# BAMresearch/McSAS

Hardware: AMD Instinct MI355X
Metric: MC accept/reject steps/sec (whole node) (higher is better)
Workload: dtype f64; 1 GPU; Sphere, synthetic 512 q-points x 400 contribs, 50 reps on this rank (50 in all), 20000 MC steps per chain per launch, convergenceCriterion=0, one analysis on the chip at a time; reps_total=50, reps_per_gpu=50, ranks_seen=1, streams=1, exec_mode=pipeline, waves_per_chain=1, q_per_lane=8, window=192, launches=108, cached_rows=True

## Files before the change

mcsas_amd/csrc/pipe_layout.h:

```cpp
#pragma once
#include "chain_common.h"

namespace mcsas {

struct PipeSnap {
    int32_t attempt, t_init, alive, pad;
    uint64_t init_base;
    uint64_t step_base;
};

struct PipeChain {
    PipeSnap snap[2];
    double SC, SIC, SCC, A, b, chi2;
    double X;
    int64_t num_iter, num_moves, total_steps;
    uint64_t draw_pos, t_start;
    int32_t attempts, converged, stopped, overflow, done, pad;
#ifdef MCSAS_STAMPS
    int64_t dbg[20];
    uint64_t last_end;
#endif
};

struct PipeGeom {
    int32_t kb;
    int32_t w;
    int32_t rows_per_wave;
    int32_t prod_blocks_y;
    int32_t scan_waves;
    int32_t qpl;
    int32_t gram_off;
    int32_t sub_per_block;
    int32_t lazy_rows;
    int32_t overlap;
    int32_t gram_lds;
    int32_t drow_off;
    int32_t resum_every;
    int32_t rowq;
    int32_t rec_off;
    int32_t help;
    uint64_t prod_lds, scan_lds;
};

struct PipeArgs {
    ChainArgs c;
    PipeGeom g;
    PipeChain *chains;
    double *ft, *wft;
    int32_t *slot_of;
    int32_t *stage_slot;
    double *dwin;
    double *gwin;
    double *scal;
    int32_t *row_valid;
    double *pval;
    int32_t *povf;
    int32_t *rowq;
    int32_t *n_done;
    int32_t *n_done_dev;
    int32_t tick, pad;
    uint64_t *timeline;
    int32_t timeline_tick, pad1;
};

struct PipeHot {
    const double *q, *w, *wI, *q3inv;
    PipeChain *chains;
    int32_t n_reps, n_contrib, n_active, qpad, kb, prod_blocks_y, w_sub, pad;
    int64_t max_iter;
};

constexpr int PIPE_BLOCK = 512;
constexpr int PIPE_WAVES = PIPE_BLOCK / 64;
constexpr int PIPE_GRAM_TILES_PER_ROUND = 2;
constexpr int PIPE_DROW_PAD = 8;
constexpr int PIPE_GRAM_NT_MAX = 3;
constexpr int PIPE_RESUM_STEPS = 64;
constexpr int PIPE_MAX_ROW_DOUBLES = 32;
#define PIPE_TL_WORDS 30

static inline int pipe_geometry(int nq, int n_contrib, int tab_doubles, int heavy_rows, int rows_per_wave_req, int sub_req, int gram_global_req, int eager_req, int n_chains, int n_cus, PipeGeom *g,
                                int contrib_doubles) {
    int qpl = 1;
    while (qpl * 64 < nq) qpl *= 2;
    if (qpl > 16) return 1;
    const int qpad = qpl * 64;
    g->rowq = 0; g->rec_off = 0; g->help = 0;
    if (heavy_rows) {
        int kb = (n_contrib / 2) & ~7;
        int cap = PIPE_BLOCK;
#ifndef __HIPCC_RTC__
        if (const char *e = getenv("MCSAS_HIP_PIPE_KB_CAP")) { const int v = atoi(e) & ~7; if (v >= 8 && v <= PIPE_BLOCK) cap = v; }
#endif
        if (kb > cap) kb = cap;
        if (n_chains > 0 && n_cus > 0) {
            const double slots = 8.0 * (double)n_cus;
            auto rate = [&](int c) { const double r = (double)n_chains * c / slots; return (double)c / (0.75 + (double)(long long)(r + 1.0 - 1e-9)); };
            const double rmax = (double)n_chains * kb / slots;
            if (rmax > 2.0 && rmax < 4.0) {
                int best = kb;
                double best_v = rate(kb);
                for (int c = kb - 8; c >= 8 && 2 * c >= kb; c -= 8)
                    if (rate(c) > best_v * 1.02) { best_v = rate(c); best = c; }
                kb = best;
            }
        }
#ifndef __HIPCC_RTC__
        if (const char *e = getenv("MCSAS_HIP_PIPE_KB")) { const int v = atoi(e) & ~7; if (v >= 8 && v <= ((n_contrib / 2) & ~7) && v <= cap) kb = v; }
#endif
        if (kb < 8) return 1;
        int by = 8;
        if (n_chains > 0 && n_cus > 0) { by = (n_cus + n_chains - 1) / n_chains; if (by < 1) by = 1; if (by > 32) by = 32; if (by * 8 > kb) by = (kb + 7) / 8; }
        g->kb = kb; g->qpl = qpl; g->w = 8; g->sub_per_block = 1; g->rows_per_wave = 1; g->prod_blocks_y = by;
        g->gram_off = 4 * qpad + tab_doubles; g->resum_every = PIPE_RESUM_STEPS;
        g->overlap = 0; g->gram_lds = 0; g->drow_off = 0; g->lazy_rows = 0;
        g->rowq = 1; g->rec_off = g->gram_off + 16;
        const size_t rec = (size_t)kb * (contrib_doubles + MCSAS_MAX_ACTIVE + 2) + ((size_t)3 * kb + 1) / 2;
        g->prod_lds = sizeof(double) * ((size_t)g->rec_off + rec);
        g->help = (n_chains > 1 && (size_t)n_chains <= 2 * rec) ? 1 : 0;
#ifndef __HIPCC_RTC__
        if (const char *e = getenv("MCSAS_HIP_PIPE_HELP")) g->help = atoi(e) ? g->help : 0;
#endif
        g->scan_waves = PIPE_WAVES;
        g->scan_lds = sizeof(double) * ((size_t)g->w * qpad + 2 * (size_t)g->w * g->w + 3 * (size_t)qpad + (size_t)g->kb * 4 + 64)
                    + sizeof(int32_t) * (4 * (size_t)g->kb + 1 + 1 + 64 + 4 + 8) + 64;
        if (g->scan_lds > 160 * 1024 || g->prod_lds > 160 * 1024) return 2;
        return 0;
    }
    const bool overlap = gram_global_req;
    auto pick_w = [&](int r) {
        int w = 8;
        for (int ws = 8; ws <= 8 * r && ws <= (overlap ? 32 : 64); ws += 8) {
            const int rps = ws / 8;
            if (rps == 5 || rps == 7 || rps * qpl > PIPE_MAX_ROW_DOUBLES) continue;
            if ((8 * r) % ws == 0 && sizeof(double) * (size_t)ws * qpad <= 96 * 1024 && (sub_req == 0 || ws <= 8 * sub_req)) w = ws;
        }
        return w;
    };
    int rpw = 0, by = 0;
    if (rows_per_wave_req >= 1 && rows_per_wave_req <= 8) {
        rpw = rows_per_wave_req;
        while (rpw > 1 && 2 * 8 * rpw > n_contrib) --rpw;
        if (2 * 8 * rpw > n_contrib) return 1;
        by = n_contrib / (2 * 8 * rpw);
        if (by * 8 * rpw > 256) by = 256 / (8 * rpw);
    } else {
        static const int order[6] = {6, 8, 4, 3, 2, 1};
        int kbs[6], best_kb = 0;
        for (int c = 0; c < 6; ++c) {
            const int r = order[c];
            int b = (2 * 8 * r > n_contrib) ? 0 : n_contrib / (2 * 8 * r);
            if (b * 8 * r > 256) b = 256 / (8 * r);
            kbs[c] = b * 8 * r;
            if (kbs[c] > best_kb) best_kb = kbs[c];
        }
        if (best_kb == 0) return 1;
        int rpw_d = 0, by_d = 0;
        for (int c = 0; c < 6 && !rpw_d; ++c)
            if (kbs[c] > 0 && 20 * kbs[c] >= 17 * best_kb) { rpw_d = order[c]; by_d = kbs[c] / (8 * rpw_d); }
        if (n_chains > 0 && n_cus > 0) {
            static const int small_first[6] = {3, 4, 6, 8, 2, 1};
            for (int c = 0; c < 6 && !rpw; ++c) {
                const int r = small_first[c];
                int b = (2 * 8 * r > n_contrib) ? 0 : n_contrib / (2 * 8 * r);
                if (b * 8 * r > 256) b = 256 / (8 * r);
                if (b > 0 && b * 8 * r == by_d * 8 * rpw_d && pick_w(r) == pick_w(rpw_d) && n_chains * (b + 1) <= n_cus) { rpw = r; by = b; }
            }
        }
        if (!rpw) { rpw = rpw_d; by = by_d; }
    }
    g->kb = by * 8 * rpw; g->qpl = qpl;
    g->w = pick_w(rpw);
    g->sub_per_block = 8 * rpw / g->w;
    g->rows_per_wave = rpw;
    g->prod_blocks_y = by;
    g->gram_off = 4 * qpad + tab_doubles;
    g->resum_every = 0;
    {
        const size_t red = overlap ? (size_t)2 * PIPE_WAVES * PIPE_GRAM_NT_MAX * 256 : (size_t)PIPE_WAVES * PIPE_GRAM_TILES_PER_ROUND * 256;
        g->prod_lds = sizeof(double) * ((size_t)g->gram_off + 16 + red);
        g->overlap = overlap ? 1 : 0;
        g->gram_lds = 0; g->drow_off = 0;
        const size_t with_rows = g->prod_lds + sizeof(double) * (size_t)g->w * (qpad + PIPE_DROW_PAD);
        if (!overlap && with_rows <= 160 * 1024) {
            g->gram_lds = 1; g->drow_off = g->gram_off + 16 + (int)red; g->prod_lds = with_rows;
        }
        g->lazy_rows = ((g->gram_lds || overlap) && !eager_req) ? 1 : 0;
        if (!g->gram_lds && !g->overlap) return 2;
#ifndef MCSAS_TUNING
        if (g->overlap) return 2;
#endif
    }
    g->scan_waves = PIPE_WAVES;
    g->scan_lds = sizeof(double) * ((size_t)g->w * qpad + 2 * (size_t)g->w * g->w + 2 * (size_t)qpad + (size_t)g->kb * 4 + 64)
                + sizeof(int32_t) * (4 * (size_t)g->kb + 1 + 1 + 64 + 4 + 8) + 64;
    if (g->scan_lds > 160 * 1024 || g->prod_lds > 160 * 1024) return 2;
    return 0;
}

}
```

mcsas_amd/csrc/pipe_prod.h:

```cpp
#pragma once
#include "pipe_rowq.h"
#include <type_traits>

namespace mcsas {

#define PIPE_PIN_ROW(arr) do { _Pragma("unroll") for (int j_ = 0; j_ < QPL; ++j_) asm volatile("" : "+v"(arr[j_])); } while (0)

#ifdef MCSAS_STAMPS
#define PIPE_TL_SLOT(pa, i) (pa).timeline[((size_t)blockIdx.x * 8 + (threadIdx.x >> 6)) * PIPE_TL_WORDS + 4 + (i)]
#define PIPE_TL_PUT(pa, t, i, val) do { if ((pa).timeline && (t) - 1 == (pa).timeline_tick && (threadIdx.x & 63) == 0) PIPE_TL_SLOT(pa, i) = (val); } while (0)
#define PIPE_TL_CLOCK(var) const uint64_t var = wall_clock64()
#else
#define PIPE_TL_PUT(pa, t, i, val) do {} while (0)
#define PIPE_TL_CLOCK(var) do {} while (0)
#endif
#define PIPE_TL_WRITE(pa, t, i) PIPE_TL_PUT(pa, t, i, wall_clock64())
#define PIPE_TLX_MARK(pa, t, i) PIPE_TL_WRITE(pa, t, 18 + (i))
#define PIPE_TL_MARK(pa, t, i) PIPE_TL_WRITE(pa, t, i)

template <int M> constexpr bool pipe_light_model_v = Contrib<M>::ROW_CLASS == 0;
template <int M>
__device__ __forceinline__ double pipe_point_intensity(const Contrib<M> &c, double q, double q3inv, const double *tab) {
    if constexpr (M == MCSAS_MODEL_SPHERE) return c.fast ? c.intensity_fast(q, q3inv) : c.intensity(q, tab);
    else return c.intensity(q, tab);
}

template <int QPL>
__device__ __forceinline__ void load_row_pairs(const MCSAS_GLOBAL double *row, int lane, double (&r)[QPL]) {
    if constexpr (QPL >= 2) {
#pragma unroll
        for (int c = 0; c < QPL / 2; ++c) {
            const v2f64 v = *(const MCSAS_GLOBAL v2f64 *)(row + 128 * c + 2 * lane);
            r[2 * c] = v.x; r[2 * c + 1] = v.y;
        }
    } else {
        r[0] = row[lane];
    }
}
template <int QPL>
__device__ __forceinline__ void load_row_pairs_lds(const double *row, int lane, double (&r)[QPL]) {
    if constexpr (QPL >= 2) {
#pragma unroll
        for (int c = 0; c < QPL / 2; ++c) {
            const v2f64 v = *reinterpret_cast<const v2f64 *>(row + 128 * c + 2 * lane);
            r[2 * c] = v.x; r[2 * c + 1] = v.y;
        }
    } else {
        r[0] = row[lane];
    }
}

template <int M, int QPL, bool RQ>
__device__ __forceinline__ void pipe_prod_block(const PipeArgs &pa, const PipeHot &hot, double *lds, int rep, int by, int gy, int t) {
    const ChainArgs &a = pa.c;
    const int tid = threadIdx.x, lane = tid & 63, wave = tid >> 6;
    constexpr int WPB = PIPE_BLOCK / 64;
    const int N = hot.n_contrib, P = hot.n_active, qpad = hot.qpad, Kb = hot.kb;
    const int64_t max_iter = hot.max_iter;
    constexpr int QTB = (QPL * 64 + PIPE_BLOCK - 1) / PIPE_BLOCK;
    double tq[QTB], tw[QTB], twI[QTB], tq3[QTB];
#pragma unroll
    for (int x = 0; x < QTB; ++x) {
        const int i = tid + PIPE_BLOCK * x < qpad ? tid + PIPE_BLOCK * x : 0;
        tq[x] = glb(hot.q)[i]; tw[x] = glb(hot.w)[i]; twI[x] = glb(hot.wI)[i]; tq3[x] = glb(hot.q3inv)[i];
    }
    PIPE_TL_CLOCK(c_entry);
    const PipeSnap sn = load_snap(&hot.chains[rep].snap[t & 1]);
    const bool own = sn.alive && t >= sn.t_init;
    if (!own && !(RQ && pa.g.help)) return;
    PIPE_TL_CLOCK(c_snap);

    double *lq = lds, *lw = lds + qpad, *lwI = lds + 2 * qpad, *lq3 = lds + 3 * qpad, *tab = lds + 4 * qpad;
#pragma unroll
    for (int x = 0; x < QTB; ++x) {
        const int i = tid + PIPE_BLOCK * x;
        if (i < qpad) { lq[i] = tq[x]; lw[i] = tw[x]; lwI[i] = twI[x]; lq3[i] = tq3[x]; }
    }
    PIPE_TL_CLOCK(c_tab);
    Contrib<M>::fill_table(a.model, tab, tid, PIPE_BLOCK);
    if (tid == 0) *reinterpret_cast<int32_t *>(lds + pa.g.gram_off + 16) = 0;
    __syncthreads();
    PIPE_TL_CLOCK(c_bar);
    PIPE_TL_PUT(pa, t, 22, c_entry); PIPE_TL_PUT(pa, t, 23, c_snap); PIPE_TL_PUT(pa, t, 24, c_tab); PIPE_TL_PUT(pa, t, 25, c_bar);
    const QTables qt = make_qtables<M>(a.model, lq, lq3, tab);
    if constexpr (RQ) { pipe_prod_rowq<M, QPL>(pa, hot, lds, qt, rep, by, gy, t, sn, own); return; }
    auto rset = glb(a.rset) + (size_t)rep * N * P;
    auto cache = glb(a.cache) + (size_t)rep * a.cache_rows * qpad;
    const DrawSource src{a.replay ? a.replay + (size_t)rep * a.replay_len : nullptr, a.replay_len, a.seed,
                         (uint32_t)(a.rep_offset + rep)};
    auto slot_of = glb(pa.slot_of) + (size_t)rep * N;
    auto stage = glb(pa.stage_slot) + (size_t)rep * 2 * Kb;
    auto row_valid = glb(pa.row_valid) + (size_t)rep * N;
    const int gw = by * WPB + wave, nw = gy * WPB;

    if (t == sn.t_init) {
        for (int i = tid + by * PIPE_BLOCK; i < N; i += PIPE_BLOCK * gy) { slot_of[i] = i; row_valid[i] = 1; }
        for (int i = tid + by * PIPE_BLOCK; i < 2 * Kb; i += PIPE_BLOCK * gy) stage[i] = N + i;
        int ovf = 0;
        for (int nb = 0; nb < N; nb += nw * WAVE) {
            const int n = nb + lane * nw + gw;
            double row[MCSAS_MAX_ACTIVE] = {0., 0., 0., 0.};
            if (n < N) {
#pragma unroll
                for (int p = 0; p < MCSAS_MAX_ACTIVE; ++p)
                    if (p < P) {
                        if (a.start_from_min) row[p] = a.start_value[p];
                        else {
                            double u = src.at(sn.init_base + (uint64_t)p * N + n, ovf);
                            row[p] = gen_transform(a.gen_kind[p], u) * (a.gen_hi[p] - a.gen_lo[p]) + a.gen_lo[p];
                        }
                        rset[(size_t)n * P + p] = row[p];
                    }
            } else {
#pragma unroll
                for (int p = 0; p < MCSAS_MAX_ACTIVE; ++p) row[p] = a.gen_lo[p] > 0. ? a.gen_lo[p] : 1e-9;
            }
            Contrib<M> mine;
            mine.prepare(a.model, row);
            for (int l = 0; l < WAVE; ++l) {
                const int nn = nb + l * nw + gw;
                if (nn >= N) break;
                const Contrib<M> c = mine.bcast(__builtin_amdgcn_readfirstlane(l));
                double it[QPL];
                RowEval<M, QPL>::run(c, qt, lane, it);
#pragma unroll
                for (int j = 0; j < QPL; ++j) cache[(size_t)nn * qpad + lane + WAVE * j] = it[j];
            }
        }
        if (__any(ovf) && lane == 0) atomicOr(&pa.chains[rep].overflow, 1);
        return;
    }

    if (MCSAS_TUNE_BITS(a) & 16) return;
    if constexpr (pipe_light_model_v<M>) if (pa.g.overlap || pa.g.gram_lds) {
        const int W = pa.g.w, nsb = pa.g.sub_per_block, BR = nsb * W;
        const int rw_even = W >> 3, skew_bits = (MCSAS_TUNE_BITS(a) >> 19) & 3;
        const int skew_req = pa.g.gram_lds ? (skew_bits == 0 ? 1 : (skew_bits == 3 ? 0 : skew_bits)) : skew_bits;
        const int skew = skew_req < rw_even ? skew_req : rw_even - 1;
        const int wv = __builtin_amdgcn_readfirstlane(wave);
        const int RW = wv < 4 ? rw_even + skew : rw_even - skew;
        const int rbase = wv < 4 ? wv * (rw_even + skew) : 4 * (rw_even + skew) + (wv - 4) * (rw_even - skew);
        const int buf = t & 1;
        const int64_t w = (int64_t)t - sn.t_init - 1;
        const int64_t sb0 = w * Kb + (int64_t)by * BR;
        auto dwin = glb(pa.dwin) + ((size_t)rep * 2 + buf) * Kb * qpad;
        auto scal = glb(pa.scal) + ((size_t)rep * 2 + buf) * Kb * 4;
        auto pval = glb(pa.pval) + ((size_t)rep * 2 + buf) * Kb * MCSAS_MAX_ACTIVE;
        auto povf = glb(pa.povf) + ((size_t)rep * 2 + buf) * Kb;
        auto gwin = glb(pa.gwin) + ((size_t)rep * 2 + buf) * Kb * W;
        double *gred = lds + pa.g.gram_off + 16;
        constexpr size_t GRED = (size_t)PIPE_WAVES * PIPE_GRAM_NT_MAX * 256;
        const int nmine = nsb * RW;
        const bool no_gram = MCSAS_TUNE_BITS(a) & 64;
        const int lrow = (lane / RW) * W + rbase + (lane % RW);
        const bool lazy = pa.g.lazy_rows;
        PIPE_TLX_MARK(pa, t, 0);
        constexpr int CON = 12;
        static_assert(sizeof(Contrib<M>) <= 8 * CON && sizeof(Contrib<M>) % 8 == 0, "Contrib record");
        int32_t *stl = reinterpret_cast<int32_t *>(gred);
        double *scon = gred + 64;
        double prow[MCSAS_MAX_ACTIVE] = {0., 0., 0., 0.};
        const int l2 = lane - 32;
        const bool old_lane = lazy && l2 >= 0 && l2 < nmine;
        int stale_r = -1;
        if (old_lane) {
            const int lrow_o = (l2 / RW) * W + rbase + (l2 % RW);
            if (sb0 + lrow_o < max_iter) {
                const int r = (int)((sb0 + lrow_o) % N);
                const int v = row_valid[r];
#pragma unroll
                for (int p = 0; p < MCSAS_MAX_ACTIVE; ++p) if (p < P) prow[p] = rset[(size_t)r * P + p];
                if (!v) stale_r = r;
            }
        }
        int pov = 0, my_oslot = 0, my_sslot = 0;
        {
            const int r = (int)((sb0 + lrow) % N);
            if (lane < nmine) {
                if (lazy) my_oslot = r;
                else { my_oslot = slot_of[r]; my_sslot = stage[buf * Kb + by * BR + lrow]; }
            }
            const int64_t sl = sb0 + lrow;
#pragma unroll
            for (int p = 0; p < MCSAS_MAX_ACTIVE; ++p)
                if (p < P) {
                    double u = 0.5;
                    if (lane < nmine && sl < max_iter) u = src.at(sn.step_base + (uint64_t)sl * P + p, pov);
                    const double pv = gen_transform(a.gen_kind[p], u) * (a.gen_hi[p] - a.gen_lo[p]) + a.gen_lo[p];
                    if (!(old_lane && sb0 + ((l2 / RW) * W + rbase + (l2 % RW)) < max_iter)) prow[p] = pv;
                }
        }
        Contrib<M> prop;
        prop.prepare(a.model, prow);
        PIPE_TLX_MARK(pa, t, 1);
        int nst = 0;
        if (lazy) {
            if (stale_r >= 0) {
                const int e = atomicAdd(&stl[0], 1);
                stl[1 + e] = stale_r;
                double tmp[CON] = {};
                __builtin_memcpy(tmp, &prop, sizeof(Contrib<M>));
#pragma unroll
                for (int i = 0; i < (int)(sizeof(Contrib<M>) / 8); ++i) scon[e * CON + i] = tmp[i];
            }
            PIPE_LDS_BARRIER();
            nst = stl[0];
            for (int i = 0; i < nst; ++i) {
                const int r = stl[1 + i];
                Contrib<M> c;
                {
                    double tmp[CON];
#pragma unroll
                    for (int x = 0; x < (int)(sizeof(Contrib<M>) / 8); ++x) tmp[x] = scon[i * CON + x];
                    __builtin_memcpy(&c, tmp, sizeof(Contrib<M>));
                }
#pragma unroll
                for (int x = 0; x < QTB; ++x) {
                    const int iq = tid + PIPE_BLOCK * x;
                    if (iq < qpad) cache[(size_t)r * qpad + iq] = pipe_point_intensity<M>(c, lq[iq], lq3[iq], tab);
                }
                if (tid == 0) row_valid[r] = 1;
            }
            if (nst) __syncthreads();
            else PIPE_LDS_BARRIER();
        }
        PIPE_TLX_MARK(pa, t, 2);
        PIPE_TLX_MARK(pa, t, 3);
        if (lane < nmine) {
            const int k = by * BR + lrow;
#pragma unroll
            for (int p = 0; p < MCSAS_MAX_ACTIVE; ++p) if (p < P) pval[k * MCSAS_MAX_ACTIVE + p] = prow[p];
            povf[k] = pov;
        }
        auto nvalid_of = [&](int ss) {
            const int64_t left = max_iter - (w * Kb + (int64_t)(by * nsb + ss) * W);
            return left >= W ? W : (left > 0 ? (int)left : 0);
        };
        if (pa.g.gram_lds) {
            const int dstr = qpad + PIPE_DROW_PAD;
            double *dbuf = lds + pa.g.drow_off;
            double ocur[QPL], onext[QPL];
            {
                const auto orow0 = cache + (size_t)__builtin_amdgcn_readlane(my_oslot, 0) * qpad + lane;
#pragma unroll
                for (int j = 0; j < QPL; ++j) ocur[j] = orow0[WAVE * j];
            }
            PIPE_PIN_ROW(ocur);
            for (int ss = 0; ss < nsb; ++ss) {
                for (int jr = 0; jr < RW; ++jr) {
                    const int l = ss * RW + jr, bl = __builtin_amdgcn_readfirstlane(l);
                    const int kl = ss * W + rbase + jr, k = by * BR + kl;
                    const Contrib<M> cnew = prop.bcast(bl);
                    const int sslot = __builtin_amdgcn_readlane(my_sslot, bl);
                    double d[QPL], nwv[QPL];
                    {
                        const int bn = __builtin_amdgcn_readfirstlane(l + 1 < nmine ? l + 1 : l);
                        const auto orow = cache + (size_t)__builtin_amdgcn_readlane(my_oslot, bn) * qpad + lane;
#pragma unroll
                        for (int j = 0; j < QPL; ++j) onext[j] = orow[WAVE * j];
                    }
                    const auto nrow = cache + (size_t)sslot * qpad + lane;
                    const auto dr = dwin + (size_t)k * qpad + lane;
                    double *dl = dbuf + (size_t)(rbase + jr) * dstr + lane;
                    RowEval<M, QPL>::run(cnew, qt, lane, nwv);
#ifdef MCSAS_STAMPS
                    if (l < 4) { PIPE_PIN_ROW(nwv); PIPE_TL_MARK(pa, t, 4 + 2 * l); }
#endif
                    PIPE_PIN_ROW(ocur); PIPE_PIN_ROW(onext); PIPE_PIN_ROW(nwv);
                    double s1 = 0., s2 = 0.;
#pragma unroll
                    for (int j = 0; j < QPL; ++j) {
                        const int iq = lane + WAVE * j;
                        if (!lazy) nrow[WAVE * j] = nwv[j];
                        d[j] = nwv[j] - ocur[j];
                        dr[WAVE * j] = d[j];
                        dl[WAVE * j] = d[j];
                        s1 = fma(lw[iq], d[j], s1); s2 = fma(lwI[iq], d[j], s2);
                    }
                    const double ae = wave_sum2_split(s1, s2, lane);
                    if (lane < 2) scal[(size_t)k * 4 + lane] = ae;
#pragma unroll
                    for (int j = 0; j < QPL; ++j) ocur[j] = onext[j];
#ifdef MCSAS_STAMPS
                    if (l < 4) PIPE_TL_MARK(pa, t, 5 + 2 * l);
#endif
                }
                PIPE_TL_MARK(pa, t, 2 * (ss < 4 ? ss : 3));
                if (!no_gram) PIPE_LDS_BARRIER();
                const int nvalid = nvalid_of(ss);
                if (nvalid > 0 && !no_gram)
                    pipe_prod_gram_lds<QPL>(dbuf, dstr, W, nvalid, lw, gred, gwin + (size_t)(by * nsb + ss) * W * W,
                                            scal + (size_t)(by * BR + ss * W) * 4);
                PIPE_TL_MARK(pa, t, 2 * (ss < 4 ? ss : 3) + 1);
            }
            PIPE_TL_MARK(pa, t, 17);
            return;
        }
#ifdef MCSAS_TUNING
#include "pipe_prod_overlap.inc"
#endif
        PIPE_TL_MARK(pa, t, 17);
        return;
    }

}

}
```

mcsas_amd/csrc/pipe_prod_overlap.inc:

```
        const int ntiles = pipe_gram_tiles(W);
        constexpr int UN = QPL;
        auto rows_and_gram = [&](auto scheme_t, auto scheme_pack) {
            constexpr int T = decltype(scheme_t)::value;
            constexpr bool PACK = decltype(scheme_pack)::value;
            constexpr int UCAP = PipeGramScheme<T, PACK>::UCAP;
            v4f64 gacc[PIPE_GRAM_NT_MAX];
            v2f64 G[PIPE_GRAM_PREF];
            for (int ss = 0; ss < nsb; ++ss) {
                const int nv_prev = ss > 0 ? nvalid_of(ss - 1) : 0;
                const bool gram_live = ss > 0 && !no_gram && nv_prev > 0;
                const auto dprev = dwin + (size_t)(by * BR + (ss > 0 ? ss - 1 : 0) * W) * qpad;
                for (int jr = 0; jr < RW; ++jr) {
                    const int l = ss * RW + jr, bl = __builtin_amdgcn_readfirstlane(l);
                    const int kl = ss * W + rbase + jr, k = by * BR + kl;
                    const Contrib<M> cnew = prop.bcast(bl);
                    const int sslot = __builtin_amdgcn_readlane(my_sslot, bl);
                    double d[QPL], nwv[QPL], ocur[QPL];
                    {
                        const auto orow = cache + (size_t)__builtin_amdgcn_readlane(my_oslot, bl) * qpad + lane;
#pragma unroll
                        for (int j = 0; j < QPL; ++j) ocur[j] = orow[WAVE * j];
                    }
                    const int u0 = (RW > 1 && jr > 0) ? UN * (jr - 1) / (RW - 1) : 0, u1 = (RW > 1 && jr > 0) ? UN * jr / (RW - 1) : 0;
                    const int npre = u1 - u0 < UCAP ? u1 - u0 : UCAP;
                    const bool chunk = gram_live && npre > 0;
                    if (chunk) pipe_gram_fetch<QPL, T, PACK>(dprev, qpad, nv_prev, wv, u0, npre, G);
                    else {
#pragma unroll
                        for (int i = 0; i < PIPE_GRAM_PREF; ++i) asm volatile("" : "=v"(G[i]));
                    }
                    const auto nrow = cache + (size_t)sslot * qpad + lane;
                    const auto dr = dwin + (size_t)k * qpad + lane;
                    RowEval<M, QPL>::run(cnew, qt, lane, nwv);
                    PIPE_PIN_ROW(ocur); PIPE_PIN_ROW(nwv);
                    if (chunk) {
                        pipe_gram_consume<QPL, T, PACK>(G, nv_prev, lw, wv, u0, npre, gacc);
                        if (u0 + npre < u1) pipe_gram_units<QPL, T, PACK>(dprev, qpad, nv_prev, lw, wv, u0 + npre, u1, gacc);
                        if (u1 == UN) pipe_gram_park(gacc, ntiles, gred + (size_t)((ss - 1) & 1) * GRED, wv, lane);
                    }
                    double s1 = 0., s2 = 0.;
#pragma unroll
                    for (int j = 0; j < QPL; ++j) {
                        const int iq = lane + WAVE * j;
                        if (!lazy) nrow[WAVE * j] = nwv[j];
                        d[j] = nwv[j] - ocur[j];
                        dr[WAVE * j] = d[j];
                        s1 = fma(lw[iq], d[j], s1); s2 = fma(lwI[iq], d[j], s2);
                    }
                    const double ae = wave_sum2_split(s1, s2, lane);
                    if (lane < 2) scal[(size_t)k * 4 + lane] = ae;
                    PIPE_TL_MARK(pa, t, (ss < 2 ? ss : 1) * 4 + (jr < 3 ? jr : 3));
                    if (ss > 0 && !no_gram && jr == 0) {
                        asm volatile("s_waitcnt vmcnt(%0)" :: "n"(QPL < 8 ? QPL : 8) : "memory");
                        PIPE_LDS_BARRIER();
                        if (ss > 1 && nvalid_of(ss - 2) > 0)
                            pipe_gram_sum_store(W, gred + (size_t)((ss - 2) & 1) * GRED, gwin + (size_t)(by * nsb + ss - 2) * W * W,
                                                scal + (size_t)(by * BR + (ss - 2) * W) * 4);
                        if (RW == 1 && nv_prev > 0) {
                            pipe_gram_units<QPL, T, PACK>(dprev, qpad, nv_prev, lw, wv, 0, UN, gacc);
                            pipe_gram_park(gacc, ntiles, gred + (size_t)((ss - 1) & 1) * GRED, wv, lane);
                        }
                    }
                }
                PIPE_TL_MARK(pa, t, 8 + (ss < 3 ? ss : 3));
            }
            if (!no_gram) {
                asm volatile("s_waitcnt vmcnt(0)" ::: "memory");
                PIPE_TL_MARK(pa, t, 12);
                PIPE_LDS_BARRIER();
                PIPE_TL_MARK(pa, t, 13);
                if (nsb > 1 && nvalid_of(nsb - 2) > 0)
                    pipe_gram_sum_store(W, gred + (size_t)((nsb - 2) & 1) * GRED, gwin + (size_t)(by * nsb + nsb - 2) * W * W,
                                        scal + (size_t)(by * BR + (nsb - 2) * W) * 4);
                const int nv = nvalid_of(nsb - 1);
                if (nv > 0) {
                    const auto dlast = dwin + (size_t)(by * BR + (nsb - 1) * W) * qpad;
                    v2f64 G2[PIPE_GRAM_PREF];
                    PIPE_TL_MARK(pa, t, 14);
                    pipe_gram_fetch<QPL, T, PACK>(dlast, qpad, nv, wv, 0, UN < UCAP ? UN : UCAP, G);
                    for (int u = 0; u < UN; u += 2 * UCAP) {
                        const int n0 = UN - u < UCAP ? UN - u : UCAP;
                        const int un = u + UCAP, n1 = un < UN ? (UN - un < UCAP ? UN - un : UCAP) : 0;
                        if (n1 > 0) pipe_gram_fetch<QPL, T, PACK>(dlast, qpad, nv, wv, un, n1, G2);
                        pipe_gram_consume<QPL, T, PACK>(G, nv, lw, wv, u, n0, gacc);
                        const int u2 = u + 2 * UCAP, n2 = u2 < UN ? (UN - u2 < UCAP ? UN - u2 : UCAP) : 0;
                        if (n2 > 0) pipe_gram_fetch<QPL, T, PACK>(dlast, qpad, nv, wv, u2, n2, G);
                        if (n1 > 0) pipe_gram_consume<QPL, T, PACK>(G2, nv, lw, wv, un, n1, gacc);
                    }
                    PIPE_TL_MARK(pa, t, 15);
                    pipe_gram_park(gacc, ntiles, gred + (size_t)((nsb - 1) & 1) * GRED, wv, lane);
                    PIPE_LDS_BARRIER();
                    PIPE_TL_MARK(pa, t, 16);
                    pipe_gram_sum_store(W, gred + (size_t)((nsb - 1) & 1) * GRED, gwin + (size_t)(by * nsb + nsb - 1) * W * W,
                                        scal + (size_t)(by * BR + (nsb - 1) * W) * 4);
                }
            }
        };
        if (W == 24) rows_and_gram(std::integral_constant<int, 2>{}, std::integral_constant<bool, true>{});
        else if (W <= 16) rows_and_gram(std::integral_constant<int, 1>{}, std::integral_constant<bool, false>{});
        else rows_and_gram(std::integral_constant<int, 2>{}, std::integral_constant<bool, false>{});
```

Baseline: 302.3 million MC steps/s.

## Replace static per-wave row assignment with LDS atomic work-claiming in gram_lds producer

In the gram_lds path, each wave no longer gets a fixed (skewed) set of rows. Waves now claim proposal rows one at a time through a workgroup-scope atomic counter in LDS. Proposal contributions and slot indices are staged in a new LDS record area, and waves read them back instead of broadcasting from lanes. This aims to balance load across waves and remove the static skew tuning. The cost is extra LDS, an atomic per row, and a barrier. The old static scheme is moved into the overlap include file.

```diff
diff --git a/mcsas_amd/csrc/pipe_layout.h b/mcsas_amd/csrc/pipe_layout.h
--- a/mcsas_amd/csrc/pipe_layout.h
+++ b/mcsas_amd/csrc/pipe_layout.h
@@ -74,6 +74,7 @@
 constexpr int PIPE_WAVES = PIPE_BLOCK / 64;
 constexpr int PIPE_GRAM_TILES_PER_ROUND = 2;
 constexpr int PIPE_DROW_PAD = 8;
+constexpr int PIPE_PROP_DOUBLES = 12;
 constexpr int PIPE_GRAM_NT_MAX = 3;
 constexpr int PIPE_RESUM_STEPS = 64;
 constexpr int PIPE_MAX_ROW_DOUBLES = 32;
@@ -181,9 +182,10 @@
         g->prod_lds = sizeof(double) * ((size_t)g->gram_off + 16 + red);
         g->overlap = overlap ? 1 : 0;
         g->gram_lds = 0; g->drow_off = 0;
-        const size_t with_rows = g->prod_lds + sizeof(double) * (size_t)g->w * (qpad + PIPE_DROW_PAD);
+        const size_t drows = (size_t)g->w * (qpad + PIPE_DROW_PAD);
+        const size_t with_rows = g->prod_lds + sizeof(double) * (drows + (size_t)8 * rpw * PIPE_PROP_DOUBLES);
         if (!overlap && with_rows <= 160 * 1024) {
-            g->gram_lds = 1; g->drow_off = g->gram_off + 16 + (int)red; g->prod_lds = with_rows;
+            g->gram_lds = 1; g->drow_off = g->gram_off + 16 + (int)red; g->rec_off = g->drow_off + (int)drows; g->prod_lds = with_rows;
         }
         g->lazy_rows = ((g->gram_lds || overlap) && !eager_req) ? 1 : 0;
         if (!g->gram_lds && !g->overlap) return 2;
diff --git a/mcsas_amd/csrc/pipe_prod.h b/mcsas_amd/csrc/pipe_prod.h
--- a/mcsas_amd/csrc/pipe_prod.h
+++ b/mcsas_amd/csrc/pipe_prod.h
@@ -78,7 +78,10 @@
     }
     PIPE_TL_CLOCK(c_tab);
     Contrib<M>::fill_table(a.model, tab, tid, PIPE_BLOCK);
-    if (tid == 0) *reinterpret_cast<int32_t *>(lds + pa.g.gram_off + 16) = 0;
+    if (tid == 0) {
+        *reinterpret_cast<int32_t *>(lds + pa.g.gram_off + 16) = 0;
+        *reinterpret_cast<int32_t *>(lds + pa.g.gram_off) = 0;
+    }
     __syncthreads();
     PIPE_TL_CLOCK(c_bar);
     PIPE_TL_PUT(pa, t, 22, c_entry); PIPE_TL_PUT(pa, t, 23, c_snap); PIPE_TL_PUT(pa, t, 24, c_tab); PIPE_TL_PUT(pa, t, 25, c_bar);
@@ -134,12 +137,6 @@
     if (MCSAS_TUNE_BITS(a) & 16) return;
     if constexpr (pipe_light_model_v<M>) if (pa.g.overlap || pa.g.gram_lds) {
         const int W = pa.g.w, nsb = pa.g.sub_per_block, BR = nsb * W;
-        const int rw_even = W >> 3, skew_bits = (MCSAS_TUNE_BITS(a) >> 19) & 3;
-        const int skew_req = pa.g.gram_lds ? (skew_bits == 0 ? 1 : (skew_bits == 3 ? 0 : skew_bits)) : skew_bits;
-        const int skew = skew_req < rw_even ? skew_req : rw_even - 1;
-        const int wv = __builtin_amdgcn_readfirstlane(wave);
-        const int RW = wv < 4 ? rw_even + skew : rw_even - skew;
-        const int rbase = wv < 4 ? wv * (rw_even + skew) : 4 * (rw_even + skew) + (wv - 4) * (rw_even - skew);
         const int buf = t & 1;
         const int64_t w = (int64_t)t - sn.t_init - 1;
         const int64_t sb0 = w * Kb + (int64_t)by * BR;
@@ -149,62 +146,24 @@
         auto povf = glb(pa.povf) + ((size_t)rep * 2 + buf) * Kb;
         auto gwin = glb(pa.gwin) + ((size_t)rep * 2 + buf) * Kb * W;
         double *gred = lds + pa.g.gram_off + 16;
-        constexpr size_t GRED = (size_t)PIPE_WAVES * PIPE_GRAM_NT_MAX * 256;
-        const int nmine = nsb * RW;
         const bool no_gram = MCSAS_TUNE_BITS(a) & 64;
-        const int lrow = (lane / RW) * W + rbase + (lane % RW);
         const bool lazy = pa.g.lazy_rows;
         PIPE_TLX_MARK(pa, t, 0);
-        constexpr int CON = 12;
-        static_assert(sizeof(Contrib<M>) <= 8 * CON && sizeof(Contrib<M>) % 8 == 0, "Contrib record");
+        constexpr int CON = PIPE_PROP_DOUBLES;
+        static_assert(sizeof(Contrib<M>) <= 8 * (CON - 1) && sizeof(Contrib<M>) % 8 == 0, "Contrib record");
         int32_t *stl = reinterpret_cast<int32_t *>(gred);
         double *scon = gred + 64;
-        double prow[MCSAS_MAX_ACTIVE] = {0., 0., 0., 0.};
-        const int l2 = lane - 32;
-        const bool old_lane = lazy && l2 >= 0 && l2 < nmine;
-        int stale_r = -1;
-        if (old_lane) {
-            const int lrow_o = (l2 / RW) * W + rbase + (l2 % RW);
-            if (sb0 + lrow_o < max_iter) {
-                const int r = (int)((sb0 + lrow_o) % N);
-                const int v = row_valid[r];
-#pragma unroll
-                for (int p = 0; p < MCSAS_MAX_ACTIVE; ++p) if (p < P) prow[p] = rset[(size_t)r * P + p];
-                if (!v) stale_r = r;
-            }
-        }
-        int pov = 0, my_oslot = 0, my_sslot = 0;
-        {
-            const int r = (int)((sb0 + lrow) % N);
-            if (lane < nmine) {
-                if (lazy) my_oslot = r;
-                else { my_oslot = slot_of[r]; my_sslot = stage[buf * Kb + by * BR + lrow]; }
-            }
-            const int64_t sl = sb0 + lrow;
-#pragma unroll
-            for (int p = 0; p < MCSAS_MAX_ACTIVE; ++p)
-                if (p < P) {
-                    double u = 0.5;
-                    if (lane < nmine && sl < max_iter) u = src.at(sn.step_base + (uint64_t)sl * P + p, pov);
-                    const double pv = gen_transform(a.gen_kind[p], u) * (a.gen_hi[p] - a.gen_lo[p]) + a.gen_lo[p];
-                    if (!(old_lane && sb0 + ((l2 / RW) * W + rbase + (l2 % RW)) < max_iter)) prow[p] = pv;
-                }
-        }
-        Contrib<M> prop;
-        prop.prepare(a.model, prow);
-        PIPE_TLX_MARK(pa, t, 1);
-        int nst = 0;
-        if (lazy) {
-            if (stale_r >= 0) {
-                const int e = atomicAdd(&stl[0], 1);
-                stl[1 + e] = stale_r;
-                double tmp[CON] = {};
-                __builtin_memcpy(tmp, &prop, sizeof(Contrib<M>));
-#pragma unroll
-                for (int i = 0; i < (int)(sizeof(Contrib<M>) / 8); ++i) scon[e * CON + i] = tmp[i];
-            }
+        auto stale_push = [&](int r, const Contrib<M> &c) {
+            const int e = atomicAdd(&stl[0], 1);
+            stl[1 + e] = r;
+            double tmp[CON] = {};
+            __builtin_memcpy(tmp, &c, sizeof(Contrib<M>));
+#pragma unroll
+            for (int i = 0; i < (int)(sizeof(Contrib<M>) / 8); ++i) scon[e * CON + i] = tmp[i];
+        };
+        auto stale_refresh = [&]() {
             PIPE_LDS_BARRIER();
-            nst = stl[0];
+            const int nst = stl[0];
             for (int i = 0; i < nst; ++i) {
                 const int r = stl[1 + i];
                 Contrib<M> c;
@@ -223,15 +182,7 @@
             }
             if (nst) __syncthreads();
             else PIPE_LDS_BARRIER();
-        }
-        PIPE_TLX_MARK(pa, t, 2);
-        PIPE_TLX_MARK(pa, t, 3);
-        if (lane < nmine) {
-            const int k = by * BR + lrow;
-#pragma unroll
-            for (int p = 0; p < MCSAS_MAX_ACTIVE; ++p) if (p < P) pval[k * MCSAS_MAX_ACTIVE + p] = prow[p];
-            povf[k] = pov;
-        }
+        };
         auto nvalid_of = [&](int ss) {
             const int64_t left = max_iter - (w * Kb + (int64_t)(by * nsb + ss) * W);
             return left >= W ? W : (left > 0 ? (int)left : 0);
@@ -239,32 +190,98 @@
         if (pa.g.gram_lds) {
             const int dstr = qpad + PIPE_DROW_PAD;
             double *dbuf = lds + pa.g.drow_off;
+            double *prec = lds + pa.g.rec_off;
+            int32_t *claim = reinterpret_cast<int32_t *>(lds + pa.g.gram_off);
+            auto take = [&]() {
+                int v = 0;
+                if (lane == 0) v = __hip_atomic_fetch_add(claim, 1, __ATOMIC_RELAXED, __HIP_MEMORY_SCOPE_WORKGROUP);
+                return __builtin_amdgcn_readfirstlane(v);
+            };
+            int kc = take();
+            const int kk = tid & 63;
+            const int64_t sl = sb0 + kk;
+            const bool prop_thr = tid < BR, old_thr = lazy && tid >= 64 && tid - 64 < BR && sl < max_iter;
+            const int rk = (int)(sl % N);
+            double prow[MCSAS_MAX_ACTIVE] = {0., 0., 0., 0.};
+            int stale_r = -1, pov = 0;
+            if (old_thr) {
+                const int v = row_valid[rk];
+#pragma unroll
+                for (int p = 0; p < MCSAS_MAX_ACTIVE; ++p) if (p < P) prow[p] = rset[(size_t)rk * P + p];
+                if (!v) stale_r = rk;
+            }
+#pragma unroll
+            for (int p = 0; p < MCSAS_MAX_ACTIVE; ++p)
+                if (p < P) {
+                    double u = 0.5;
+                    if (prop_thr && sl < max_iter) u = src.at(sn.step_base + (uint64_t)sl * P + p, pov);
+                    const double pv = gen_transform(a.gen_kind[p], u) * (a.gen_hi[p] - a.gen_lo[p]) + a.gen_lo[p];
+                    if (!old_thr) prow[p] = pv;
+                }
+            Contrib<M> prop;
+            prop.prepare(a.model, prow);
+            PIPE_TLX_MARK(pa, t, 1);
+            if (prop_thr) {
+                double tmp[CON] = {};
+                __builtin_memcpy(tmp, &prop, sizeof(Contrib<M>));
+#pragma unroll
+                for (int i = 0; i < (int)(sizeof(Contrib<M>) / 8); ++i) prec[kk * CON + i] = tmp[i];
+                if (!lazy) {
+                    int32_t *slots = reinterpret_cast<int32_t *>(prec + kk * CON + CON - 1);
+                    slots[0] = slot_of[rk]; slots[1] = stage[buf * Kb + by * BR + kk];
+                }
+                const int k = by * BR + kk;
+#pragma unroll
+                for (int p = 0; p < MCSAS_MAX_ACTIVE; ++p) if (p < P) pval[k * MCSAS_MAX_ACTIVE + p] = prow[p];
+                povf[k] = pov;
+            }
+            if (stale_r >= 0) stale_push(stale_r, prop);
+            if (lazy) stale_refresh();
+            else PIPE_LDS_BARRIER();
+            PIPE_TLX_MARK(pa, t, 2);
+            PIPE_TLX_MARK(pa, t, 3);
+            const int r0 = (int)(sb0 % N);
+            auto oslot_of = [&](int k) {
+                if (lazy) return r0 + k < N ? r0 + k : r0 + k - N;
+                return __builtin_amdgcn_readfirstlane(reinterpret_cast<const int32_t *>(prec + k * CON + CON - 1)[0]);
+            };
             double ocur[QPL], onext[QPL];
             {
-                const auto orow0 = cache + (size_t)__builtin_amdgcn_readlane(my_oslot, 0) * qpad + lane;
+                const auto orow0 = cache + (size_t)oslot_of(kc < BR ? kc : BR - 1) * qpad + lane;
 #pragma unroll
                 for (int j = 0; j < QPL; ++j) ocur[j] = orow0[WAVE * j];
             }
             PIPE_PIN_ROW(ocur);
+#ifdef MCSAS_STAMPS
+            int nmine = 0;
+#endif
             for (int ss = 0; ss < nsb; ++ss) {
-                for (int jr = 0; jr < RW; ++jr) {
-                    const int l = ss * RW + jr, bl = __builtin_amdgcn_readfirstlane(l);
-                    const int kl = ss * W + rbase + jr, k = by * BR + kl;
-                    const Contrib<M> cnew = prop.bcast(bl);
-                    const int sslot = __builtin_amdgcn_readlane(my_sslot, bl);
+                while (kc < (ss + 1) * W) {
+                    const int kn = take();
+                    const int k = by * BR + kc;
+                    Contrib<M> cnew;
+                    int sslot = 0;
+                    {
+                        Contrib<M> cl;
+                        double tmp[CON];
+#pragma unroll
+                        for (int i = 0; i < (int)(sizeof(Contrib<M>) / 8); ++i) tmp[i] = prec[kc * CON + i];
+                        __builtin_memcpy(&cl, tmp, sizeof(Contrib<M>));
+                        cnew = cl.bcast(0);
+                        if (!lazy) sslot = __builtin_amdgcn_readfirstlane(reinterpret_cast<const int32_t *>(prec + kc * CON + CON - 1)[1]);
+                    }
                     double d[QPL], nwv[QPL];
                     {
-                        const int bn = __builtin_amdgcn_readfirstlane(l + 1 < nmine ? l + 1 : l);
-                        const auto orow = cache + (size_t)__builtin_amdgcn_readlane(my_oslot, bn) * qpad + lane;
+                        const auto orow = cache + (size_t)oslot_of(kn < BR ? kn : kc) * qpad + lane;
 #pragma unroll
                         for (int j = 0; j < QPL; ++j) onext[j] = orow[WAVE * j];
                     }
                     const auto nrow = cache + (size_t)sslot * qpad + lane;
                     const auto dr = dwin + (size_t)k * qpad + lane;
-                    double *dl = dbuf + (size_t)(rbase + jr) * dstr + lane;
+                    double *dl = dbuf + (size_t)(kc - ss * W) * dstr + lane;
                     RowEval<M, QPL>::run(cnew, qt, lane, nwv);
 #ifdef MCSAS_STAMPS
-                    if (l < 4) { PIPE_PIN_ROW(nwv); PIPE_TL_MARK(pa, t, 4 + 2 * l); }
+                    if (nmine < 4) { PIPE_PIN_ROW(nwv); PIPE_TL_MARK(pa, t, 4 + 2 * nmine); }
 #endif
                     PIPE_PIN_ROW(ocur); PIPE_PIN_ROW(onext); PIPE_PIN_ROW(nwv);
                     double s1 = 0., s2 = 0.;
@@ -282,8 +299,10 @@
 #pragma unroll
                     for (int j = 0; j < QPL; ++j) ocur[j] = onext[j];
 #ifdef MCSAS_STAMPS
-                    if (l < 4) PIPE_TL_MARK(pa, t, 5 + 2 * l);
-#endif
+                    if (nmine < 4) PIPE_TL_MARK(pa, t, 5 + 2 * nmine);
+                    ++nmine;
+#endif
+                    kc = kn;
                 }
                 PIPE_TL_MARK(pa, t, 2 * (ss < 4 ? ss : 3));
                 if (!no_gram) PIPE_LDS_BARRIER();
diff --git a/mcsas_amd/csrc/pipe_prod_overlap.inc b/mcsas_amd/csrc/pipe_prod_overlap.inc
--- a/mcsas_amd/csrc/pipe_prod_overlap.inc
+++ b/mcsas_amd/csrc/pipe_prod_overlap.inc
@@ -1,3 +1,55 @@
+        const int wv = __builtin_amdgcn_readfirstlane(wave);
+        const int rw_even = W >> 3, skew_req = (MCSAS_TUNE_BITS(a) >> 19) & 3;
+        const int skew = skew_req < rw_even ? skew_req : rw_even - 1;
+        const int RW = wv < 4 ? rw_even + skew : rw_even - skew;
+        const int rbase = wv < 4 ? wv * (rw_even + skew) : 4 * (rw_even + skew) + (wv - 4) * (rw_even - skew);
+        constexpr size_t GRED = (size_t)PIPE_WAVES * PIPE_GRAM_NT_MAX * 256;
+        const int nmine = nsb * RW;
+        const int lrow = (lane / RW) * W + rbase + (lane % RW);
+        double prow[MCSAS_MAX_ACTIVE] = {0., 0., 0., 0.};
+        const int l2 = lane - 32;
+        const bool old_lane = lazy && l2 >= 0 && l2 < nmine;
+        int stale_r = -1;
+        if (old_lane) {
+            const int lrow_o = (l2 / RW) * W + rbase + (l2 % RW);
+            if (sb0 + lrow_o < max_iter) {
+                const int r = (int)((sb0 + lrow_o) % N);
+                const int v = row_valid[r];
+#pragma unroll
+                for (int p = 0; p < MCSAS_MAX_ACTIVE; ++p) if (p < P) prow[p] = rset[(size_t)r * P + p];
+                if (!v) stale_r = r;
+            }
+        }
+        int pov = 0, my_oslot = 0, my_sslot = 0;
+        {
+            const int r = (int)((sb0 + lrow) % N);
+            if (lane < nmine) {
+                if (lazy) my_oslot = r;
+                else { my_oslot = slot_of[r]; my_sslot = stage[buf * Kb + by * BR + lrow]; }
+            }
+            const int64_t sl = sb0 + lrow;
+#pragma unroll
+            for (int p = 0; p < MCSAS_MAX_ACTIVE; ++p)
+                if (p < P) {
+                    double u = 0.5;
+                    if (lane < nmine && sl < max_iter) u = src.at(sn.step_base + (uint64_t)sl * P + p, pov);
+                    const double pv = gen_transform(a.gen_kind[p], u) * (a.gen_hi[p] - a.gen_lo[p]) + a.gen_lo[p];
+                    if (!(old_lane && sb0 + ((l2 / RW) * W + rbase + (l2 % RW)) < max_iter)) prow[p] = pv;
+                }
+        }
+        Contrib<M> prop;
+        prop.prepare(a.model, prow);
+        PIPE_TLX_MARK(pa, t, 1);
+        if (stale_r >= 0) stale_push(stale_r, prop);
+        if (lazy) stale_refresh();
+        PIPE_TLX_MARK(pa, t, 2);
+        PIPE_TLX_MARK(pa, t, 3);
+        if (lane < nmine) {
+            const int k = by * BR + lrow;
+#pragma unroll
+            for (int p = 0; p < MCSAS_MAX_ACTIVE; ++p) if (p < P) pval[k * MCSAS_MAX_ACTIVE + p] = prow[p];
+            povf[k] = pov;
+        }
         const int ntiles = pipe_gram_tiles(W);
         constexpr int UN = QPL;
         auto rows_and_gram = [&](auto scheme_t, auto scheme_pack) {
```

New measurement: 308.9 million MC steps/s, median of 6. 1.02x the previous value.
